# andrekuros/Multi-UAV-TA-gym-env

Hardware: AMD Instinct MI355X
Metric: env-steps/sec at N parallel envs, WPS_hard 16x32; 1/2/4/8 GPU (higher is better)
Workload: dtype f64

## Files before the change

include/muavta.h:

```cpp
#ifndef MUAVTA_H
#define MUAVTA_H

#include <stddef.h>
#include <stdint.h>

#ifdef __cplusplus
extern "C" {
#endif

#define MUAVTA_ABI_VERSION 1

enum { MUAVTA_R1 = 0, MUAVTA_R2 = 1, MUAVTA_E1 = 2, MUAVTA_F1 = 3, MUAVTA_F2 = 4, MUAVTA_T1 = 5, MUAVTA_T2 = 6 };
enum { MUAVTA_HOLD = 0, MUAVTA_REC = 1, MUAVTA_ATT = 2, MUAVTA_DEF = 3, MUAVTA_INT = 4, MUAVTA_DET = 5 };
enum { MUAVTA_EV_RESET_ALLOCATION = 0, MUAVTA_EV_NEW_THREAT = 1, MUAVTA_EV_AGENT_FAIL = 2,
       MUAVTA_EV_ESCORT_CREATED = 3, MUAVTA_EV_ESCORT_RETIRED = 4 };

enum {
  MUAVTA_OK = 0,
  MUAVTA_E_ARG = -1,
  MUAVTA_E_NO_DEVICE = -2,
  MUAVTA_E_HIP = -3,
  MUAVTA_E_CAPACITY = -4,
  MUAVTA_E_STATE = -5
};
// ... 194 lines not shown
  int32_t* n_stepped; uint8_t* park; double* reward_sum;
  int32_t max_steps, reserved;
} MuavtaRlRun;
int muavta_rl_run_device(MuavtaEnv* env, const MuavtaRlRun* run);
int muavta_step_run(MuavtaEnv* env, const int32_t* act_agent, const int32_t* act_index, int32_t gate, int32_t replan_interval, int32_t max_steps,
                    int32_t write_obs, int32_t* n_stepped, uint8_t* park, double* reward_sum);

int muavta_rollout(MuavtaEnv* env, const uint64_t* seeds, int32_t n_steps, int32_t replan_interval,
                   int32_t use_visibility, int32_t write_obs);

int muavta_set_lanes(MuavtaEnv* env, int32_t lanes);
int muavta_lanes(const MuavtaEnv* env, int32_t* mode, int32_t* allocated);
int muavta_rollout_metrics_back(MuavtaEnv* env, int32_t back, double* out);
int muavta_error_flags_back(MuavtaEnv* env, int32_t back, int32_t* flags );

int muavta_set_slot_cap(MuavtaEnv* env, int32_t cap);

int muavta_observe(MuavtaEnv* env, float* tasks, uint64_t* legal, uint8_t* pad, float* agents, float* flags);

int muavta_step_result(MuavtaEnv* env, double* reward, uint8_t* done);

int muavta_metrics(MuavtaEnv* env, double* out);

int muavta_get(MuavtaEnv* env, MuavtaField field, void* dst, size_t bytes);
int muavta_set(MuavtaEnv* env, MuavtaField field, const void* src, size_t bytes);

int muavta_get_state(MuavtaEnv* env, void* dst, size_t bytes);
int muavta_set_state(MuavtaEnv* env, const void* src, size_t bytes);

int muavta_lsap(int32_t device, const double* cost, int32_t n, int32_t nr, int32_t nc, int64_t* row, int64_t* col);
// ... 53 lines not shown
```

multi-uav-ta-gym-env_amd/batched.py:

```python
from __future__ import annotations

import ctypes as C
from typing import Optional, Sequence

import numpy as np

from . import native
from .native import MuavtaError
from .params import METRIC_KEYS, N_METRICS, N_SCALARS, MuavtaDims, MuavtaParams, params_from_config

F = {name: i for i, name in enumerate([
    "AGENT_POS", "AGENT_STATE", "AGENT_HEAD", "AGENT_QUEUE", "AGENT_NFT", "AGENT_NFP", "AGENT_CAPS", "AGENT_ATTACK_CAP",
    "AGENT_TYPE", "AGENT_NAME_IDX", "AGENT_DIST", "AGENT_MISC", "TASK_ID", "TASK_STATUS", "TASK_POS", "TASK_CUR",
    "TASK_ALLOC", "TASK_ORG_DONE", "TASK_META", "TASK_TIMES", "KNOWN", "THREAT_POS", "THREAT_META", "SCALARS",
    "OPEN_IDS", "EVENTS", "EVENT_LIST", "STAGED_ACTIONS", "ERROR", "RELEASE_LOG", "KNOWN_COUNT", "ESCORTS"])}


def _vp(a: Optional[np.ndarray]):
    return None if a is None else a.ctypes.data_as(C.c_void_p)


def _fp(a: np.ndarray):
    return C.c_void_p(a.ctypes.data)

# ... 589 lines not shown
        self._ck(self.L.muavta_metrics(self.h, _vp(m)))
        return m

    def set_slot_cap(self, cap: int = 0):
        self._ck(self.L.muavta_set_slot_cap(self.h, int(cap)))
        self.slot_cap = int(cap)

    def set_lanes(self, lanes: int = 0):
        self._ck(self.L.muavta_set_lanes(self.h, int(lanes)))

    def lanes(self):
        m, a = C.c_int32(), C.c_int32()
        self._ck(self.L.muavta_lanes(self.h, C.byref(m), C.byref(a)))
        return int(m.value), int(a.value)

    def error_flags(self, back: int = 0) -> np.ndarray:
        out = np.empty(self.n_envs, dtype=np.int32)
        self._ck(self.L.muavta_error_flags_back(self.h, int(back), _vp(out)))
        return out

    def rollout_metrics(self, back: int = 0) -> np.ndarray:
        m = np.empty((self.n_envs, N_METRICS), dtype=np.float64)
        if back:
            self._ck(self.L.muavta_rollout_metrics_back(self.h, int(back), _vp(m)))
            return m
        self._ck(self.L.muavta_rollout_metrics(self.h, _vp(m)))
        if self._esc_rows:
            for i, row in self._esc_rows.items():
                m[i] = row
        return m
# ... 129 lines not shown
```

multi-uav-ta-gym-env_amd/csrc/muavta_device.h:

```cpp
#pragma once
#include <hip/hip_runtime.h>
#include <cstddef>
#include <type_traits>

#include "muavta_state.h"

#define DEV __device__ __forceinline__
#define DEVN __device__ __noinline__

#ifndef MUAVTA_PACE_PRIO
#define MUAVTA_PACE_PRIO 4
#endif
#ifndef MUAVTA_PACE_HOLD
#define MUAVTA_PACE_HOLD 0
#endif
#ifndef MUAVTA_PACE_HOLD_WINDOW
#define MUAVTA_PACE_HOLD_WINDOW 48
#endif
#ifndef MUAVTA_PACE_HOLD_SLEEP
#define MUAVTA_PACE_HOLD_SLEEP 16
#endif
#ifndef MUAVTA_PACE_HOLD_POLLS
#define MUAVTA_PACE_HOLD_POLLS 256
#endif
// ... 94 lines not shown
  DEV unsigned long long* prof_lds() { return reinterpret_cast<unsigned long long*>(reinterpret_cast<unsigned char*>(&X) + sizeof(Scratch<TL>)); }
  DEV void prof_begin() { if (threadIdx.x < PROF_N) prof_lds()[threadIdx.x] = 0; if (threadIdx.x == 0) prof_lds()[PROF_N] = clock64(); lds_sync(); }
  DEV void prof_flush(int env) { lds_sync(); if (threadIdx.x < PROF_N && (g_prof_target < 0 || g_prof_target == env)) atomicAdd(&g_prof[threadIdx.x], prof_lds()[threadIdx.x]); }
#endif
  enum { A = TL::A, T = TL::T, H = TL::H, R = TL::R, E = TL::E, Q = TL::Q, KW = TL::KW };
  typedef EnvCold<TL> Cold;
  State& S;
  Cold& C;
  Scratch<TL>& X;
  double* rel_log = nullptr;
  const int32_t* more_agent = nullptr;
  const int32_t* more_index = nullptr;
  int more_cap = 0, more_pos = 0;
  int tnow;
  const DevParams& P;
  uint32_t* tape;
  int lane;
  const uint32_t* win_ptr;
  uint32_t win_len, win_stride;
  bool in_step = false;

  __device__ Sim(State& s, Cold& c, Scratch<TL>& x, const DevParams& p, uint32_t* t)
      : S(s), C(c), X(x), P(p), tape(t), lane(opaque_lane()), win_ptr(&s.rng_win[0][0]), win_len(8), win_stride(8), tnow(s.time_steps) {}
  static __device__ __forceinline__ int opaque_lane() {
    int l = threadIdx.x;
    asm volatile("" : "+v"(l));
    return l;
  }
  DEV void sync_clock() { tnow = S.time_steps; }
  DEV QueueSide<A, T, true>& qs() const {
    if constexpr (TL::SLIM) return static_cast<QueueSide<A, T, true>&>(C); else return static_cast<QueueSide<A, T, true>&>(S);
  }

  DEV void fail(int code) { if (S.error == 0) S.error = code; }
  enum { OBS_STATIC = 1 << 16 };
  DEV void obs_static_clear() { const int v = S.obs_rows; if (v > 0) S.obs_rows = v & (OBS_STATIC - 1); }
  DEV double speed_of(int t) const {
    return t == 0 ? P.speed[0] : t == 1 ? P.speed[1] : t == 2 ? P.speed[2] : t == 3 ? P.speed[3] : t == 4 ? P.speed[4]
         : t == 5 ? P.speed[5] : P.speed[6];
  }


#include "sim/rng.inc"
#include "sim/entities.inc"
#include "sim/reset.inc"
#include "sim/step.inc"
// ... 15 lines not shown
```

multi-uav-ta-gym-env_amd/csrc/muavta_kernels.hip:

```cpp
#include <hip/hip_runtime.h>
#include <dlfcn.h>
#include <rccl/rccl.h>

#include <cmath>
#include <cstdio>
#include <cstdlib>
#include <cstring>
#include <new>
#include <string>
#include <vector>

#include "muavta_device.h"

using namespace muavta;

namespace {

#define AS1 __attribute__((address_space(1)))
#define AS3 __attribute__((address_space(3)))
#define AS4 __attribute__((address_space(4)))
template <class T> __device__ __forceinline__ T* as_global(T* p) { return (T*)(AS1 T*)p; }

struct ObsPtrs {
  float* tasks;
// ... 14 lines not shown
  uint32_t* pace;
  PairPolicyDev pol;
};
enum { PACE_KEYS = 1 << 16 };
__device__ __forceinline__ const DevCtx& ctx_ref(const DevCtx* p) {
  const uint64_t b = (uint64_t)p;
  const uint32_t lo = __builtin_amdgcn_readfirstlane((uint32_t)b), hi = __builtin_amdgcn_readfirstlane((uint32_t)(b >> 32));
  return *(const DevCtx*)(const AS4 DevCtx*)(((uint64_t)hi << 32) | lo);
}
__device__ __forceinline__ ObsPtrs obs_ptrs(const DevCtx& c) {
  ObsPtrs o;
  o.tasks = as_global(c.O.tasks); o.legal = as_global(c.O.legal); o.pad = as_global(c.O.pad); o.agents = as_global(c.O.agents);
  o.flags = as_global(c.O.flags); o.reward = as_global(c.O.reward); o.done = as_global(c.O.done);
  return o;
}
template <class TL> __device__ __forceinline__ EnvState<TL>* blob_of(const DevCtx& c, int env) { return as_global(reinterpret_cast<EnvState<TL>*>(c.blobs)) + env; }
template <class TL> __device__ __forceinline__ EnvCold<TL>* cold_of(const DevCtx& c, int env) { return as_global(reinterpret_cast<EnvCold<TL>*>(c.cold)) + env; }
__device__ __forceinline__ uint32_t* tape_of(const DevCtx& c, int env) { return as_global(c.tapes) + (size_t)env * MUAVTA_RNG_STREAMS * MUAVTA_RNG_WORDS; }

template <class TL>
__device__ __forceinline__ void obs_for_env(Sim<TL>& sim, const DevParams& P, const ObsPtrs& O, int env, bool handle_buffer = true) {
  const size_t mt = (size_t)P.max_tasks, nA = (size_t)P.n_agents;
  sim.write_obs(O.tasks + (size_t)env * mt * 21, O.legal + (size_t)env * nA * ((mt + 63) >> 6), O.pad + (size_t)env * mt,
                O.agents + (size_t)env * nA * 9, O.flags + (size_t)env * 5, handle_buffer);
  if (threadIdx.x == 0) {
    O.reward[env] = sim.S.last_reward;
    O.done[env] = (uint8_t)((sim.S.terminated ? 1 : 0) | (sim.S.truncated ? 2 : 0));
  }
}

__device__ __forceinline__ void copy16(void* dst, const void* src, int bytes) {
// ... 16 lines not shown

#define smem muavta_smem
#ifdef MUAVTA_PROF
#define PROF_AT(sim, i) do { if (threadIdx.x == 0) { unsigned long long t_ = clock64(); (sim).prof_lds()[i] += t_ - (sim).prof_lds()[PROF_N]; (sim).prof_lds()[PROF_N] = t_; } } while (0)
#define PROF_EXTRA_LDS MUAVTA_PROF_LDS_BYTES
#else
#define PROF_AT(sim, i) do { } while (0)
#define PROF_EXTRA_LDS 0
#endif
#if MUAVTA_LDS_ZERO_REG
static __device__ __forceinline__ uint32_t lds_zero() { uint32_t z; asm volatile("v_mov_b32 %0, 0" : "=v"(z)); return z; }
#else
static __device__ __forceinline__ uint32_t lds_zero() { return 0u; }
#endif
#define KERNEL_LDS(TL) __shared__ __align__(16) unsigned char lds_own[Lds<TL>::bytes() + PROF_EXTRA_LDS]
static_assert(Lds<Tile16>::bytes() <= 10240, "Tile16 no longer fits 16 workgroups per CU");
static_assert(!MUAVTA_TILE24_SLIM || Lds<Tile24>::bytes() <= 10240, "Tile24 no longer fits 16 workgroups per CU");
static_assert(sizeof(EnvState<Tile16>) % 16 == 0 && sizeof(EnvState<Tile24>) % 16 == 0 && sizeof(EnvState<Tile64>) % 16 == 0, "blob copies move 16 B per lane");
static_assert(sizeof(EnvCold<Tile16>) % 16 == 0 && sizeof(EnvCold<Tile24>) % 16 == 0 && sizeof(EnvCold<Tile64>) % 16 == 0, "cold records are 16 B aligned");

#ifdef MUAVTA_MIN_WAVES
#define TILE_MIN_WAVES(TL) MUAVTA_MIN_WAVES
#else
#define TILE_MIN_WAVES(TL) TL::MIN_WAVES
#endif

struct GenrandTable {
  uint32_t v[624];
  constexpr GenrandTable() : v{} {
    uint32_t g = 19650218u;
    v[0] = g;
// ... 301 lines not shown
        if (G.R.reward_sum) as_global(G.R.reward_sum)[env] = rsum;
      }
      break;
    }
  }
  lds_sync();
  copy16(blob, L.S, sizeof(EnvState<TL>));
}

#ifndef MUAVTA_PHASE_ATTR
#define MUAVTA_PHASE_ATTR __forceinline__
#define MUAVTA_PHASE_INLINED 1
#else
#define MUAVTA_PHASE_INLINED 0
#endif
enum { PH_ALLOC = 1, PH_STEP = 2, PH_OBS = 4 };
template <class TL>
struct RecordPtrs {
  typename Sim<TL>::TokPtrs K;
  double* s_wps;
  ObsPtrs O;
  int n_envs;
};
struct RecBlob { uint32_t w[64]; };
__global__ void k_store_rec(RecBlob b, uint32_t* dst) { dst[threadIdx.x] = b.w[threadIdx.x]; }

template <class TL, bool REC, bool BL = false, bool PM = false>
__device__ MUAVTA_PHASE_ATTR void rollout_phase(const DevCtx* ctxp, unsigned char* lds_own, uint32_t lds_base, int env, int phases, int interval, int use_vis, int mode,
                                                const RecordPtrs<TL>& rec, int slot, int oslot) {
  const DevCtx& ctx = ctx_ref(ctxp);
#if MUAVTA_PHASE_INLINED
  Lds<TL> L(lds_own + lds_zero());
#else
  Lds<TL> L((unsigned char*)(AS3 unsigned char*)(uintptr_t)__builtin_amdgcn_readfirstlane(lds_base));
#endif
  Sim<TL> sim(*L.S, *cold_of<TL>(ctx, env), *L.X, ctx.P, tape_of(ctx, env));
  if (phases & PH_STEP) sim.step(true);
  if (phases & PH_OBS) {
    ObsPtrs O = obs_ptrs(ctx);
    int at = env;
    bool handle_buffer = true;
    if constexpr (REC) {
      if (oslot >= 0) {
        handle_buffer = false;
        O.tasks = as_global(rec.O.tasks); O.legal = as_global(rec.O.legal); O.pad = as_global(rec.O.pad); O.agents = as_global(rec.O.agents);
        O.flags = as_global(rec.O.flags); O.reward = as_global(rec.O.reward); O.done = as_global(rec.O.done);
        at = oslot * rec.n_envs + env;
      }
    }
    obs_for_env(sim, ctx.P, O, at, handle_buffer);
  }
// ... 3 lines not shown
                                       reinterpret_cast<unsigned char*>(L.S) + Lds<TL>::bytes() + PROF_EXTRA_LDS);
    else if constexpr (BL) sim.allocate_baseline(interval, use_vis, mode);
    else sim.allocate(interval, use_vis, mode);
    if (REC && rec.K.task_feats) {
      const typename Sim<TL>::TokPtrs K = global_tok_ptrs<TL>(rec.K);
      cold_sync();
      sim.tokens(K, slot * rec.n_envs + env);
      if (threadIdx.x == 0) as_global(rec.s_wps)[(size_t)slot * rec.n_envs + env] = sim.s_wps();
      lds_sync();
    }
  }
  PROF_AT(sim, 20);
}

template <class TL, bool REC, bool BL = false, bool PM = false>
__global__ __launch_bounds__(WG, PM ? (TILE_MIN_WAVES(TL) < 3 ? TILE_MIN_WAVES(TL) : 3) : TILE_MIN_WAVES(TL)) void k_rollout(const DevCtx* __restrict__ ctxp, const uint64_t* seeds, int n_steps, int interval, int use_vis,
                                                int mode, int write_obs, double* metrics, const uint32_t* seedbuf, const RecordPtrs<TL>* __restrict__ recp, int epoch, int env_base) {
  const DevCtx& ctx = ctx_ref(ctxp);
  const uint32_t rec_lo = __builtin_amdgcn_readfirstlane((uint32_t)(uint64_t)recp), rec_hi = __builtin_amdgcn_readfirstlane((uint32_t)((uint64_t)recp >> 32));
  const RecordPtrs<TL>& rec = *(const RecordPtrs<TL>*)(const AS4 RecordPtrs<TL>*)(((uint64_t)rec_hi << 32) | (uint64_t)rec_lo);
  const int env = env_base + blockIdx.x;
  __shared__ __align__(16) unsigned char lds_own[Lds<TL>::bytes() + PROF_EXTRA_LDS + (PM ? SCORED_EXTRA_LDS : 0)];
  Lds<TL> L(lds_own);
  EnvState<TL>* blob = blob_of<TL>(ctx, env);
  Sim<TL> sim(*L.S, *cold_of<TL>(ctx, env), *L.X, ctx.P, tape_of(ctx, env));
#ifndef MUAVTA_PACE_SCOPE
#if MUAVTA_PACE_HOLD
#define MUAVTA_PACE_SCOPE __HIP_MEMORY_SCOPE_AGENT
#else
#define MUAVTA_PACE_SCOPE __HIP_MEMORY_SCOPE_WORKGROUP
#endif
#endif
static_assert(MUAVTA_PACE_HOLD_POLLS > 0 && MUAVTA_PACE_HOLD_POLLS <= (1 << 16), "the hold loop of the pacing block must be poll-bounded");
#ifndef MUAVTA_PACE_EVERY
#define MUAVTA_PACE_EVERY 1
#endif
#if MUAVTA_PACE_PRIO
  constexpr bool PACED = TL::A <= 32 && !ABL(10);
  const uint32_t hw_id = __builtin_amdgcn_s_getreg(4 | (31 << 11)), xcc_id = __builtin_amdgcn_s_getreg(20 | (3 << 11));
  uint32_t* pace_row = as_global(ctx.pace) + ((((xcc_id & 15u) << 12) | ((hw_id >> 4) & 0xFFFu)) << 4);
// ... 24 lines not shown
          if (rec.K.task_feats) {
            const typename Sim<TL>::TokPtrs K = global_tok_ptrs<TL>(rec.K);
            const double fin = sim.s_wps();
            for (int sl = k - 1; sl < n_steps; sl++) {
              sim.tokens_pad(K, sl * rec.n_envs + env);
              if (threadIdx.x == 0) as_global(rec.s_wps)[(size_t)sl * rec.n_envs + env] = fin;
            }
          }
        }
        k = n_steps;
        continue;
      }
      ph = PH_STEP | (write_obs ? PH_OBS : 0) | (k < n_steps ? PH_ALLOC : 0);
    } else ph = (write_obs && !(REC && rec.O.tasks)) ? 0 : PH_OBS;
#if MUAVTA_PACE_PRIO
    uint32_t seen = 0;
    if (PACED && k >= 1 && k <= n_steps && (k & (MUAVTA_PACE_EVERY - 1)) == 0) {
      if (threadIdx.x == 0) __hip_atomic_store(pace_row + (hw_id & 15u), pace_tag | (uint32_t)k, __ATOMIC_RELAXED, MUAVTA_PACE_SCOPE);
      if (threadIdx.x < 16) seen = __hip_atomic_load(pace_row + threadIdx.x, __ATOMIC_RELAXED, MUAVTA_PACE_SCOPE);
    }
#endif
    if (ph) rollout_phase<TL, REC, BL, PM>(ctxp, lds_own, lds_base, env, ph, interval, use_vis, mode, rec, k < n_steps ? k : n_steps,
                                   (REC && rec.O.tasks && k >= 1 && k <= n_steps) ? k - 1 : -1);
#if MUAVTA_PACE_PRIO
    if (PACED && k >= 1 && k <= n_steps && (k & (MUAVTA_PACE_EVERY - 1)) == 0) {
      const bool behind_me = threadIdx.x < 16 && (seen >> 16) == (uint32_t)epoch && (seen & 0xFFFFu) < (uint32_t)k;
#if MUAVTA_PACE_PRIO == 4
      const int n_behind = __popcll(__ballot(behind_me));
      if (n_behind == 0) __builtin_amdgcn_s_setprio(3); else if (n_behind == 1) __builtin_amdgcn_s_setprio(2);
      else if (n_behind == 2) __builtin_amdgcn_s_setprio(1); else __builtin_amdgcn_s_setprio(0);
#else
      if (__ballot(behind_me) != 0ull) __builtin_amdgcn_s_setprio(0); else __builtin_amdgcn_s_setprio(MUAVTA_PACE_PRIO);
#endif
#if MUAVTA_PACE_HOLD
      for (int polls = 0; polls < MUAVTA_PACE_HOLD_POLLS; polls++) {
        const uint32_t st = seen & 0xFFFFu;
        const bool wait_for = threadIdx.x < 16 && (seen >> 16) == (uint32_t)epoch && st + MUAVTA_PACE_HOLD < (uint32_t)k &&
                              st + MUAVTA_PACE_HOLD_WINDOW >= (uint32_t)k;
        if (__ballot(wait_for) == 0ull) break;
        __builtin_amdgcn_s_sleep(MUAVTA_PACE_HOLD_SLEEP);
        if (threadIdx.x < 16) seen = __hip_atomic_load(pace_row + threadIdx.x, __ATOMIC_RELAXED, MUAVTA_PACE_SCOPE);
      }
#endif
    }
#endif
  }
#if MUAVTA_PACE_PRIO
  if (PACED && threadIdx.x == 0) __hip_atomic_store(pace_row + (hw_id & 15u), pace_tag | 0xFFFFu, __ATOMIC_RELAXED, MUAVTA_PACE_SCOPE);
  __builtin_amdgcn_s_setprio(0);
#endif
  if (REC && rec.K.task_feats) {
    if (threadIdx.x == 0) as_global(rec.s_wps)[(size_t)n_steps * rec.n_envs + env] = sim.s_wps();
  }
  sim.sync_clock();
  sim.metrics(as_global(metrics) + (size_t)env * MUAVTA_N_METRICS);
  lds_sync();
  copy16(blob, L.S, sizeof(EnvState<TL>));
#ifdef MUAVTA_PROF
  sim.prof_flush(env);
#endif
#ifdef MUAVTA_DIAG_TIMES
  if (threadIdx.x == 0 && env < 65536) {
    as_global(ctx.pace)[(1u << 19) + 65536 + env] = (uint32_t)__builtin_amdgcn_s_memrealtime();
    as_global(ctx.pace)[(1u << 19) + 131072 + env] = __builtin_amdgcn_s_getreg(4 | (31 << 11)) | (__builtin_amdgcn_s_getreg(20 | (3 << 11)) << 16);
  }
#endif
}

template <class TL>
__global__ __launch_bounds__(WG) void k_metrics(const DevCtx* __restrict__ ctxp, double* metrics) {
// ... 320 lines not shown
extern "C" int muavta_set_parts(MuavtaEnv* e, int32_t n_parts);
extern "C" int muavta_set_release_log(MuavtaEnv* e, int32_t enable);
extern "C" int muavta_create(const MuavtaParams* params, int32_t n_envs, int32_t device, MuavtaEnv** out);
extern "C" int muavta_destroy(MuavtaEnv* e);
extern "C" int muavta_set_slot_cap(MuavtaEnv* e, int32_t cap);
static int push_policy(MuavtaEnv* lane, const MuavtaEnv::HandleLevel& hl);

namespace {

template <class TL>
int launch_attr(MuavtaEnv* e) {
  size_t lds = Lds<TL>::bytes();
  e->lds_bytes = lds;
  if (lds > 48 * 1024) {
    const void* ks[] = {reinterpret_cast<const void*>(&k_reset<TL>), reinterpret_cast<const void*>(&k_step<TL>), reinterpret_cast<const void*>(&k_allocate<TL>),
                        reinterpret_cast<const void*>(&k_rollout<TL, false>), reinterpret_cast<const void*>(&k_rollout<TL, true>), reinterpret_cast<const void*>(&k_metrics<TL>), reinterpret_cast<const void*>(&k_observe<TL>),
                        reinterpret_cast<const void*>(&k_tokens<TL>), reinterpret_cast<const void*>(&k_call<TL>), reinterpret_cast<const void*>(&k_context<TL>),
                        reinterpret_cast<const void*>(&k_allocate<TL, true>), reinterpret_cast<const void*>(&k_rollout<TL, false, true>),
                        reinterpret_cast<const void*>(&k_pair_scores<TL>), reinterpret_cast<const void*>(&k_rollout<TL, false, false, true>)};
    for (const void* k : ks) HIPCHK(e, hipFuncSetAttribute(k, hipFuncAttributeMaxDynamicSharedMemorySize, (int)lds));
    HIPCHK(e, hipFuncSetAttribute(reinterpret_cast<const void*>(&k_allocate<TL, false, true>), hipFuncAttributeMaxDynamicSharedMemorySize, (int)lds + SCORED_EXTRA_LDS));
    HIPCHK(e, hipFuncSetAttribute(reinterpret_cast<const void*>(&k_allocate_scored<TL>), hipFuncAttributeMaxDynamicSharedMemorySize, (int)lds + SCORED_EXTRA_LDS));
  }
  return MUAVTA_OK;
}

#define DISPATCH(e, CALL)                    \
  switch ((e)->tile) {                       \
    case TK16: { typedef Tile16 TL; CALL; } break; \
    case TK24: { typedef Tile24 TL; CALL; } break; \
    default:   { typedef Tile64 TL; CALL; } break; \
// ... 870 lines not shown
    R.n_envs = e->n_envs;
    static_assert(sizeof(RecordPtrs<TL>) <= MuavtaEnv::REC_SLOT, "record-pointer slot too small");
    RecBlob blob;
    memset(&blob, 0, sizeof(blob));
    memcpy(&blob, &R, sizeof(R));
    hipLaunchKernelGGL(k_store_rec, dim3(1), dim3(64), 0, stream, blob, (uint32_t*)((char*)e->d_rec + MuavtaEnv::REC_SLOT));
    hipLaunchKernelGGL((k_rollout<TL, true>), dim3(n_launch), dim3(WG), extra_lds, stream, (const DevCtx*)e->d_ctx, ds,
                       n_steps, interval, use_vis, e->alloc_mode, write_obs, e->d_metrics, sb, (const RecordPtrs<TL>*)((char*)e->d_rec + MuavtaEnv::REC_SLOT), epoch, env_base);
  } else if (e->alloc_mode == MUAVTA_ALLOC_MLP_PAIR) {
    hipLaunchKernelGGL((k_rollout<TL, false, false, true>), dim3(n_launch), dim3(WG), extra_lds, stream, (const DevCtx*)e->d_ctx, ds,
                       n_steps, interval, use_vis, e->alloc_mode, write_obs, e->d_metrics, sb, (const RecordPtrs<TL>*)e->d_rec, epoch, env_base);
  } else if (e->alloc_mode >= MUAVTA_ALLOC_CAP_GREEDY) {
    hipLaunchKernelGGL((k_rollout<TL, false, true>), dim3(n_launch), dim3(WG), extra_lds, stream, (const DevCtx*)e->d_ctx, ds,
                       n_steps, interval, use_vis, e->alloc_mode, write_obs, e->d_metrics, sb, (const RecordPtrs<TL>*)e->d_rec, epoch, env_base);
  } else {
    hipLaunchKernelGGL((k_rollout<TL, false>), dim3(n_launch), dim3(WG), extra_lds, stream, (const DevCtx*)e->d_ctx, ds,
                       n_steps, interval, use_vis, e->alloc_mode, write_obs, e->d_metrics, sb, (const RecordPtrs<TL>*)e->d_rec, epoch, env_base);
  }
}
extern "C" {
static int rollout_impl(MuavtaEnv* e, const uint64_t* seeds, int32_t n_steps, int32_t interval, int32_t use_vis, int32_t write_obs, const MuavtaRecord* rec) {
  if (!e || n_steps < 0) return MUAVTA_E_ARG;
  if (!seeds && !e->did_reset) { e->err = "rollout without seeds before reset"; return MUAVTA_E_STATE; }
  DeviceScope scope_(e->device);
  if (seeds && e->hl.lanes_mode != 1) {
    bool want = e->hl.lanes_mode == 2;
    if (!want && e->n_rollouts) { want = hipEventQuery(e->ev1[(e->n_rollouts - 1) % MuavtaEnv::EV_RING]) == hipErrorNotReady; (void)hipGetLastError(); }
    if (want && ensure_twin(e) == MUAVTA_OK) flip_lanes(e);
  }
  MAIN_OP(e);
  const uint64_t* ds = nullptr;
  const uint32_t* sb = nullptr;
// ... 781 lines not shown
  if (lanes == 2) { int rc = ensure_twin(e); if (rc) { e->err = "muavta_set_lanes: the second lane could not be created: " + g_create_error; return rc; } }
  if (lanes == 1 && e->hl.twin) {
    muavta_destroy(e->hl.twin);
    e->hl.twin = nullptr;
  }
  e->hl.lanes_mode = lanes;
  return MUAVTA_OK;
}
int muavta_lanes(const MuavtaEnv* e, int32_t* mode, int32_t* allocated) {
  if (!e) return MUAVTA_E_ARG;
  if (mode) *mode = e->hl.lanes_mode;
  if (allocated) *allocated = e->hl.twin ? 2 : 1;
  return MUAVTA_OK;
}

int muavta_lsap(int32_t device, const double* cost, int32_t n, int32_t nr, int32_t nc, int64_t* row, int64_t* col) {
  return muavta_lsap_impl(device, cost, n, nr, nc, row, col, MUAVTA_LSAP_AUTO);
}
int muavta_lsap_impl(int32_t device, const double* cost, int32_t n, int32_t nr, int32_t nc, int64_t* row, int64_t* col, int32_t impl) {
  int ndev = 0;
  if (hipGetDeviceCount(&ndev) != hipSuccess || ndev < 1) { g_create_error = "muavta_lsap: no HIP device"; return MUAVTA_E_NO_DEVICE; }
  if (!cost || !row || !col || n < 1 || nr < 1 || nc < 1) { g_create_error = "muavta_lsap: bad arguments"; return MUAVTA_E_ARG; }
  int mn = nr < nc ? nr : nc, mx = nr < nc ? nc : nr;
  if (mn > Tile64::A || mx > Tile64::T) { g_create_error = "muavta_lsap: at most 64 x 128"; return MUAVTA_E_ARG; }
  for (size_t i = 0, m = (size_t)n * nr * nc; i < m; i++)
    if (std::isnan(cost[i]) || cost[i] == -INFINITY) { g_create_error = "muavta_lsap: matrix contains invalid numeric entries (NaN or -inf)"; return MUAVTA_E_ARG; }
  const bool fits_reg = mn <= TileLsapReg::A && mx <= TileLsapReg::T;
  if (impl < MUAVTA_LSAP_AUTO || impl > MUAVTA_LSAP_REGISTERS || (impl == MUAVTA_LSAP_REGISTERS && !fits_reg)) {
    g_create_error = "muavta_lsap_impl: unknown solver, or problem beyond 32 x 64 for the register solver"; return MUAVTA_E_ARG;
  }
// ... 112 lines not shown
```

multi-uav-ta-gym-env_amd/csrc/muavta_state.h:

```cpp
#pragma once
#include <stdint.h>

#include "../../include/muavta.h"


enum {
  MUAVTA_ERR_NONE = 0,
  MUAVTA_ERR_TASK_SLOTS = 1,
  MUAVTA_ERR_QUEUE = 2,
  MUAVTA_ERR_EVENTS = 3,
  MUAVTA_ERR_PENDING = 4,
  MUAVTA_ERR_POSITION = 5,
  MUAVTA_ERR_ESCORTS = 6,
  MUAVTA_ERR_LSAP = 7,
};

enum { TF_ESCORT = 1, TF_COUNTED = 2, TF_REACHED = 4, TF_ELIGIBLE = 8, TF_DEADLINE = 16,
       TF_KNOWN_ALL = 32  };

struct DevParams {
  int32_t n_agents, n_tasks , max_tasks , n_threats;
  int32_t n_agent_groups, agent_type[MUAVTA_MAX_GROUPS], agent_count[MUAVTA_MAX_GROUPS];
  int32_t n_task_groups, task_type[MUAVTA_MAX_GROUPS], task_count[MUAVTA_MAX_GROUPS];
  int32_t n_threat_groups, threat_type[MUAVTA_MAX_GROUPS], threat_count[MUAVTA_MAX_GROUPS];
// ... 3 lines not shown
      escort_required_agents , commit_horizon;
  uint32_t escort_mask;
  double speed[7];
  double threat_prob;
  double reward_norm_factor;
  double sense_sq_bound;
  double fail_rate, arrival_rate, dynamic_idle_penalty, sense_radius, miss_penalty, on_time_bonus,
      reassign_penalty, escort_radius, escort_requirement, escort_intercept_radius, mutual_support_radius;
  double rw[8];
  double escort_sq_bound;
  double inv_mts, inv_max_tasks;
  int32_t slot_cap;
  int32_t rw_plain;
};

template <int A_, int T_, int H_, int R_, int E_, int Q_, bool REGC_ = false, bool OTFC_ = false, bool SLIM_ = false>
struct Tile {
  static constexpr bool SLIM = SLIM_;
  static constexpr bool REGC = REGC_;
  static constexpr bool OTFC = OTFC_;
  static constexpr bool NO_COST_TILE = REGC_ || OTFC_;
  static constexpr int A = A_;
  static constexpr int T = T_;
  static constexpr int H = H_;
  static constexpr int R = R_;
  static constexpr int E = E_;
  static constexpr int Q = Q_;
  static constexpr int KW = (T_ + 31) / 32;
  static constexpr int MIN_WAVES = A_ > 32 ? 2 : 4;
  static_assert(A_ <= 64 && T_ <= 128 && H_ <= 64, "ids of agents / slots / threats are stored in int8");
};

// ... 4 lines not shown
template <> struct BucketMask<16> { typedef uint32_t type; };
template <> struct BucketMask<24> { typedef uint32_t type; };

typedef int8_t i8;
typedef int16_t i16;
typedef uint8_t u8;

template <int A, int T, bool HERE> struct QueueSide {
  double a_nfx[A], a_nfy[A], a_nft[A];
  double t_org[T], t_done[T];
  double area[3][3];
};
template <int A, int T> struct QueueSide<A, T, false> {};

template <class TL>
struct alignas(16) EnvCold : QueueSide<TL::A, TL::T, TL::SLIM> {
  enum { A = TL::A, T = TL::T, Q = TL::Q };
  double t_cur[6][T], t_alloc[6][T];
  double t_init[T], t_dtime[T];
  double a_qtime[A][Q];
  double obst[8][3];
};

template <class TL>
struct alignas(16) EnvState : QueueSide<TL::A, TL::T, !TL::SLIM> {
  enum { A = TL::A, T = TL::T, H = TL::H, R = TL::R, E = TL::E, Q = TL::Q, KW = TL::KW };
  double a_px[A], a_py[A];
  double a_dist[A];
  double a_caps[6][A];
  double t_px[T], t_py[T];
  double h_px[H], h_py[H];
// ... 42 lines not shown
      idle_reserve_steps, burst_region_toggle, escort_requests, escort_completed, escort_failed,
      escort_required_steps, escort_covered_steps, protection_breaches, threats_intercepted, recon_losses,
      escort_losses, mutual_support_engagements, protected_rec_completed;
  int32_t pending_reset, terminated, truncated, error, did_reset;
  int32_t last_plan_step, n_replans, n_calls;
  int32_t gate_step;
  uint32_t rng_idx[4];
  uint32_t rng_win[4][8];
  uint32_t rng_win_at[4];
  int32_t times_dirty;
  int32_t obs_rows;
  int32_t list_stale;
};

typedef Tile<16, 40, 16, 48, 40, 10, true> Tile16;
#ifndef MUAVTA_TILE24_SLIM
#define MUAVTA_TILE24_SLIM 1
#endif
typedef Tile<24, 48, 24, 88, 32, 12, true, false, MUAVTA_TILE24_SLIM != 0> Tile24;
typedef Tile<64, 128, 48, 128, 96, 12, true, true> Tile64;

#define MUAVTA_REL_ROW 29
#define MUAVTA_RNG_STREAMS 4
#define MUAVTA_RNG_WORDS 1248
```

multi-uav-ta-gym-env_amd/csrc/sim/entities.inc:

```
  DEV bool ref_valid(int id, int slot) const { return slot >= 0 && S.t_id[slot] == id; }
  DEV bool ref_retired(int id, int slot) const { return !ref_valid(id, slot) || S.t_status[slot] == 2; }
  DEV int head_id(int a) const { return S.a_qlen[a] > 0 ? S.a_qid[a][0] : 0; }
  DEV int queue_find(int a, int id) const {
    const int n = S.a_qlen[a];
    unsigned m = 0;
#pragma unroll
    for (int k = 0; k < Q; k++) m |= (unsigned)(S.a_qid[a][k] == id) << k;
    m &= (1u << n) - 1u;
    return m ? __ffs((int)m) - 1 : -1;
  }
  DEV void queue_erase(int a, int k) {
    const int n = S.a_qlen[a];
    for (int i = k; i + 1 < n; i++) {
      S.a_qid[a][i] = S.a_qid[a][i + 1];
      S.a_qslot[a][i] = S.a_qslot[a][i + 1];
    }
    for (int i = k; i + 1 < n; i += 4) {
      const int r = n - 1 - i;
      double t0 = 0, t1 = 0, t2 = 0, t3 = 0;
      if (r >= 1) t0 = C.a_qtime[a][i + 1];
      if (r >= 2) t1 = C.a_qtime[a][i + 2];
      if (r >= 3) t2 = C.a_qtime[a][i + 3];
      if (r >= 4) t3 = C.a_qtime[a][i + 4];
      if (r >= 1) C.a_qtime[a][i] = t0;
// ... 611 lines not shown
            }
          }
        }
      }
    }
    lds_sync();
    return __ballot(chg) != 0ull;
  }

  DEV void norm_vector(double& x, double& y) {
    double m = norm2(x, y);
    if (m == 0) { x = 0; y = 0; return; }
    const double r = frcp_nr(m);
    x = fdiv_r(x, m, r); y = fdiv_r(y, m, r);
  }
  DEV void avoid_obstacles(double px, double py, double mx, double my, double& ax, double& ay) {
    ax = 0.0; ay = 0.0;
    const double PI = 3.14159265358979323846;
    for (int o = 0; o < P.num_obstacles; o++) {
      double dx = C.obst[o][0] - px, dy = C.obst[o][1] - py;
      double d_zone = sqrt(dx * dx + dy * dy) - C.obst[o][2];
      if (d_zone < 40.0) {
        double nx = dx / d_zone, ny = dy / d_zone;
        double force = libm_log(fmax(1.05, d_zone));
        force = 0.5 / (1.0 - force);
        double ang = libm_atan2(my, mx) - libm_atan2(dy, dx);
        ang = fmod(ang + PI, 2.0 * PI) - PI;
        double rx, ry;
        if (ang > 0.0) { rx = ny; ry = -nx; } else { rx = -ny; ry = nx; }
        ax += rx * force;
        ay += ry * force;
      }
    }
  }
  DEV void random_position(int st, double min_distance, double own_range, bool contact_line, int area, bool check_obs,
                           double& ox, double& oy) {
    double limit_line = contact_line ? CONTACT_LINE : 0;
    for (int tries = 0; tries < 100; tries++) {
      double x, y;
      if (area >= 0) {
        double tlx = qs().area[area][0], tly = qs().area[area][1], w = qs().area[area][2];
// ... 57 lines not shown
```

multi-uav-ta-gym-env_amd/native.py:

```python
from __future__ import annotations

import ctypes as C
import os
import sys
import shutil
import subprocess

from .params import MuavtaDims, MuavtaParams

PKG_DIR = os.path.dirname(os.path.abspath(__file__))
CSRC = os.path.join(PKG_DIR, "csrc")
SO_PATH = os.environ.get("MUAVTA_SO") or os.path.join(PKG_DIR, "libmuavta.so")
HIPCC_FLAGS = ["--offload-arch=gfx950", "-O3", "-ldl", "-mllvm", "-disable-machine-licm",
                "-ffp-contract=off", "-std=c++17", "-fPIC", "-shared", "-Wno-unused-value", "-Wno-invalid-offsetof"]

EXPORTS = [
    "muavta_create", "muavta_destroy", "muavta_last_error", "muavta_dims", "muavta_reset", "muavta_step",
    "muavta_allocate", "muavta_step_staged", "muavta_rollout", "muavta_observe", "muavta_step_result",
    "muavta_metrics", "muavta_get", "muavta_set", "muavta_get_state", "muavta_set_state", "muavta_lsap",
    "muavta_avoid_obstacles", "muavta_device_ptrs", "muavta_last_kernel_ms", "muavta_sync",
    "muavta_rollout_metrics", "muavta_refresh_observation", "muavta_get_rng", "muavta_set_rng", "muavta_abi_sizes",
    "muavta_set_allocator", "muavta_tokens", "muavta_tokens_device", "muavta_set_release_log", "muavta_lsap_impl",
    "muavta_last_seed_ms", "muavta_call", "muavta_rollout_record", "muavta_comm_uid", "muavta_comm_init", "muavta_allreduce_metrics", "muavta_comm_destroy",
    "muavta_kernel_ms_history", "muavta_wait_stream", "muavta_set_parts", "muavta_part_range", "muavta_rollout_part", "muavta_allocate_part",
    "muavta_step_part", "muavta_observe_part", "muavta_wait_part", "muavta_domain_math", "muavta_domain_log", "muavta_domain_atan2", "muavta_step_lists",
    "muavta_allocate_scored", "muavta_allocate_scored_device", "muavta_rl_step_device", "muavta_launch_gaps_ms",
    "muavta_rl_run_device", "muavta_step_run", "muavta_set_lanes", "muavta_lanes", "muavta_rollout_metrics_back", "muavta_error_flags_back", "muavta_set_slot_cap", "muavta_context", "muavta_context_device",
    "muavta_set_pair_policy", "muavta_pair_scores", "muavta_pair_scores_device",
]


class MuavtaError(RuntimeError):
    pass


class MuavtaScored(C.Structure):
    _fields_ = [("kind", C.c_int32), ("max_tasks", C.c_int32), ("max_agents", C.c_int32), ("gate", C.c_int32), ("flags", C.c_int32),
                ("replan_interval", C.c_int32), ("use_visibility", C.c_int32), ("reserved0", C.c_int32),
                ("edge_scores", C.c_void_p), ("task_pri", C.c_void_p), ("reserved", C.c_void_p), ("selected", C.c_void_p),
                ("replanned", C.c_void_p)]


class MuavtaPairMlp(C.Structure):
# ... 116 lines not shown
    L.muavta_tokens.argtypes = [vp, i32, i32, i32] + [vp] * 10
    L.muavta_tokens_device.argtypes = [vp, i32, i32, i32] + [vp] * 10
    L.muavta_allocate_scored.argtypes = [vp, C.POINTER(MuavtaScored), vp, vp]
    L.muavta_allocate_scored_device.argtypes = [vp, C.POINTER(MuavtaScored)]
    L.muavta_rl_step_device.argtypes = [vp, C.POINTER(MuavtaRlStep)]
    L.muavta_rl_run_device.argtypes = [vp, C.POINTER(MuavtaRlRun)]
    L.muavta_step_run.argtypes = [vp, vp, vp, i32, i32, i32, i32, vp, vp, vp]
    L.muavta_set_lanes.argtypes = [vp, i32]
    L.muavta_set_slot_cap.argtypes = [vp, i32]
    L.muavta_context.argtypes = [vp, i32, i32, vp]
    L.muavta_context_device.argtypes = [vp, i32, i32, vp]
    L.muavta_set_pair_policy.argtypes = [vp, C.POINTER(MuavtaPairMlp)]
    L.muavta_pair_scores.argtypes = [vp, vp, vp]
    L.muavta_pair_scores_device.argtypes = [vp, vp, vp]
    L.muavta_lanes.argtypes = [vp, C.POINTER(i32), C.POINTER(i32)]
    L.muavta_rollout_metrics_back.argtypes = [vp, i32, vp]
    L.muavta_error_flags_back.argtypes = [vp, i32, vp]
    L.muavta_abi_sizes.argtypes = [C.POINTER(i32 * 3)]
    for name in EXPORTS:
        if name != "muavta_last_error":
            getattr(L, name).restype = C.c_int
    sizes = (i32 * 3)()
    L.muavta_abi_sizes(C.byref(sizes))
    if (sizes[0], sizes[1]) != (C.sizeof(MuavtaParams), C.sizeof(MuavtaDims)):
        raise MuavtaError(f"ABI layout mismatch: library {sizes[0]}/{sizes[1]} bytes vs binding "
                          f"{C.sizeof(MuavtaParams)}/{C.sizeof(MuavtaDims)} (MuavtaParams/MuavtaDims)")
    _LIB = L
    return L
```

Before: 236.6 million.

## Add lean Tile16 rollout with QueueSide in global memory for higher occupancy

Adds a Tile16Lean variant for the plain rollout kernel that keeps the QueueSide portion of env state in the global blob instead of LDS. This shrinks per-workgroup LDS so more workgroups fit per CU, and raises the launch-bounds minimum waves to 5. Queue accesses now go to global memory, which adds latency. It also computes the two atan2 calls in a nounroll loop to shrink code, moves the pace-row loads to after the phase, and adds an occupancy query API.

```diff
diff --git a/include/muavta.h b/include/muavta.h
--- a/include/muavta.h
+++ b/include/muavta.h
@@ -232,6 +232,8 @@
 int muavta_rollout_metrics_back(MuavtaEnv* env, int32_t back, double* out);
 int muavta_error_flags_back(MuavtaEnv* env, int32_t back, int32_t* flags );
 
+int muavta_rollout_occupancy(MuavtaEnv* env, int32_t* workgroups_per_cu);
+
 int muavta_set_slot_cap(MuavtaEnv* env, int32_t cap);
 
 int muavta_observe(MuavtaEnv* env, float* tasks, uint64_t* legal, uint8_t* pad, float* agents, float* flags);
diff --git a/multi-uav-ta-gym-env_amd/batched.py b/multi-uav-ta-gym-env_amd/batched.py
--- a/multi-uav-ta-gym-env_amd/batched.py
+++ b/multi-uav-ta-gym-env_amd/batched.py
@@ -627,6 +627,13 @@
         self._ck(self.L.muavta_lanes(self.h, C.byref(m), C.byref(a)))
         return int(m.value), int(a.value)
 
+    def rollout_occupancy(self) -> int:
+        if not hasattr(self.L, "muavta_rollout_occupancy"):
+            raise MuavtaError("this build of libmuavta.so has no muavta_rollout_occupancy")
+        n = C.c_int32()
+        self._ck(self.L.muavta_rollout_occupancy(self.h, C.byref(n)))
+        return int(n.value)
+
     def error_flags(self, back: int = 0) -> np.ndarray:
         out = np.empty(self.n_envs, dtype=np.int32)
         self._ck(self.L.muavta_error_flags_back(self.h, int(back), _vp(out)))
diff --git a/multi-uav-ta-gym-env_amd/csrc/muavta_device.h b/multi-uav-ta-gym-env_amd/csrc/muavta_device.h
--- a/multi-uav-ta-gym-env_amd/csrc/muavta_device.h
+++ b/multi-uav-ta-gym-env_amd/csrc/muavta_device.h
@@ -132,6 +132,7 @@
   int more_cap = 0, more_pos = 0;
   int tnow;
   const DevParams& P;
+  QueueSide<A, T, true>* QB = nullptr;
   uint32_t* tape;
   int lane;
   const uint32_t* win_ptr;
@@ -140,14 +141,22 @@
 
   __device__ Sim(State& s, Cold& c, Scratch<TL>& x, const DevParams& p, uint32_t* t)
       : S(s), C(c), X(x), P(p), tape(t), lane(opaque_lane()), win_ptr(&s.rng_win[0][0]), win_len(8), win_stride(8), tnow(s.time_steps) {}
+  __device__ Sim(State& s, Cold& c, Scratch<TL>& x, const DevParams& p, uint32_t* t, int lane_)
+      : S(s), C(c), X(x), P(p), tape(t), lane(lane_), win_ptr(&s.rng_win[0][0]), win_len(8), win_stride(8), tnow(s.time_steps) {}
   static __device__ __forceinline__ int opaque_lane() {
     int l = threadIdx.x;
     asm volatile("" : "+v"(l));
     return l;
   }
+  static __device__ __forceinline__ uint32_t wave_lane() {
+    uint32_t l = __builtin_amdgcn_mbcnt_hi(~0u, __builtin_amdgcn_mbcnt_lo(~0u, 0u));
+    asm volatile("" : "+v"(l));
+    return l;
+  }
   DEV void sync_clock() { tnow = S.time_steps; }
   DEV QueueSide<A, T, true>& qs() const {
-    if constexpr (TL::SLIM) return static_cast<QueueSide<A, T, true>&>(C); else return static_cast<QueueSide<A, T, true>&>(S);
+    if constexpr (TL::LEAN) return *(QueueSide<A, T, true>*)(__attribute__((address_space(1))) QueueSide<A, T, true>*)QB;
+    else if constexpr (TL::SLIM) return static_cast<QueueSide<A, T, true>&>(C); else return static_cast<QueueSide<A, T, true>&>(S);
   }
 
   DEV void fail(int code) { if (S.error == 0) S.error = code; }
diff --git a/multi-uav-ta-gym-env_amd/csrc/muavta_kernels.hip b/multi-uav-ta-gym-env_amd/csrc/muavta_kernels.hip
--- a/multi-uav-ta-gym-env_amd/csrc/muavta_kernels.hip
+++ b/multi-uav-ta-gym-env_amd/csrc/muavta_kernels.hip
@@ -52,7 +52,15 @@
   o.flags = as_global(c.O.flags); o.reward = as_global(c.O.reward); o.done = as_global(c.O.done);
   return o;
 }
-template <class TL> __device__ __forceinline__ EnvState<TL>* blob_of(const DevCtx& c, int env) { return as_global(reinterpret_cast<EnvState<TL>*>(c.blobs)) + env; }
+template <class TL> __device__ __forceinline__ EnvState<TL>* blob_of(const DevCtx& c, int env) {
+  if constexpr (TL::LEAN) {
+    typedef EnvState<typename TL::Full> FS;
+    return reinterpret_cast<EnvState<TL>*>(reinterpret_cast<unsigned char*>(as_global(reinterpret_cast<FS*>(c.blobs)) + env) + offsetof(FS, a_px));
+  } else return as_global(reinterpret_cast<EnvState<TL>*>(c.blobs)) + env;
+}
+template <class TL> __device__ __forceinline__ QueueSide<TL::A, TL::T, true>* qs_of(const DevCtx& c, int env) {
+  return reinterpret_cast<QueueSide<TL::A, TL::T, true>*>(as_global(reinterpret_cast<EnvState<typename TL::Full>*>(c.blobs)) + env);
+}
 template <class TL> __device__ __forceinline__ EnvCold<TL>* cold_of(const DevCtx& c, int env) { return as_global(reinterpret_cast<EnvCold<TL>*>(c.cold)) + env; }
 __device__ __forceinline__ uint32_t* tape_of(const DevCtx& c, int env) { return as_global(c.tapes) + (size_t)env * MUAVTA_RNG_STREAMS * MUAVTA_RNG_WORDS; }
 
@@ -99,7 +107,22 @@
 static __device__ __forceinline__ uint32_t lds_zero() { return 0u; }
 #endif
 #define KERNEL_LDS(TL) __shared__ __align__(16) unsigned char lds_own[Lds<TL>::bytes() + PROF_EXTRA_LDS]
+static_assert(Lds<Tile16Lean>::bytes() <= 8192, "the plain rollout of Tile16 no longer fits 20 workgroups per CU");
 static_assert(Lds<Tile16>::bytes() <= 10240, "Tile16 no longer fits 16 workgroups per CU");
+template <class TL> struct LeanImage {
+  typedef typename TL::Full FT;
+  static constexpr size_t offset() { return offsetof(EnvState<FT>, a_px); }
+  static constexpr bool ok() {
+    return offsetof(EnvState<TL>, a_px) == 0 && offset() % 8 == 0 && offset() + sizeof(EnvState<TL>) <= sizeof(EnvState<FT>) &&
+           offsetof(EnvState<FT>, list_stale) - offset() == offsetof(EnvState<TL>, list_stale) &&
+           offsetof(EnvState<FT>, esc_mask) - offset() == offsetof(EnvState<TL>, esc_mask) &&
+           offsetof(EnvState<FT>, a_qslot) - offset() == offsetof(EnvState<TL>, a_qslot) &&
+           offsetof(EnvState<FT>, t_bucket) - offset() == offsetof(EnvState<TL>, t_bucket) &&
+           sizeof(EnvCold<TL>) == sizeof(EnvCold<FT>) && offsetof(EnvCold<TL>, obst) == offsetof(EnvCold<FT>, obst) &&
+           sizeof(QueueSide<TL::A, TL::T, true>) <= offset();
+  }
+};
+static_assert(LeanImage<Tile16Lean>::ok(), "Tile16Lean is not the image of Tile16 behind QueueSide");
 static_assert(!MUAVTA_TILE24_SLIM || Lds<Tile24>::bytes() <= 10240, "Tile24 no longer fits 16 workgroups per CU");
 static_assert(sizeof(EnvState<Tile16>) % 16 == 0 && sizeof(EnvState<Tile24>) % 16 == 0 && sizeof(EnvState<Tile64>) % 16 == 0, "blob copies move 16 B per lane");
 static_assert(sizeof(EnvCold<Tile16>) % 16 == 0 && sizeof(EnvCold<Tile24>) % 16 == 0 && sizeof(EnvCold<Tile64>) % 16 == 0, "cold records are 16 B aligned");
@@ -431,6 +454,13 @@
 #else
 #define MUAVTA_PHASE_INLINED 0
 #endif
+template <class TL> struct RolloutTile { typedef TL type; };
+template <> struct RolloutTile<Tile16> { typedef Tile16Lean type; };
+#ifdef MUAVTA_MIN_WAVES
+#define ROLLOUT_MIN_WAVES(TL, REC, BL, PM) ((PM) && MUAVTA_MIN_WAVES > 3 ? 3 : MUAVTA_MIN_WAVES)
+#else
+#define ROLLOUT_MIN_WAVES(TL, REC, BL, PM) ((PM) ? (TL::MIN_WAVES < 3 ? TL::MIN_WAVES : 3) : TL::LEAN ? 5 : TL::MIN_WAVES)
+#endif
 enum { PH_ALLOC = 1, PH_STEP = 2, PH_OBS = 4 };
 template <class TL>
 struct RecordPtrs {
@@ -451,7 +481,9 @@
 #else
   Lds<TL> L((unsigned char*)(AS3 unsigned char*)(uintptr_t)__builtin_amdgcn_readfirstlane(lds_base));
 #endif
-  Sim<TL> sim(*L.S, *cold_of<TL>(ctx, env), *L.X, ctx.P, tape_of(ctx, env));
+  constexpr bool FIVE = ROLLOUT_MIN_WAVES(TL, REC, BL, PM) > TL::MIN_WAVES;
+  Sim<TL> sim(*L.S, *cold_of<TL>(ctx, env), *L.X, ctx.P, tape_of(ctx, env), FIVE ? (int)Sim<TL>::wave_lane() : Sim<TL>::opaque_lane());
+  if constexpr (TL::LEAN) sim.QB = qs_of<TL>(ctx, env);
   if (phases & PH_STEP) sim.step(true);
   if (phases & PH_OBS) {
     ObsPtrs O = obs_ptrs(ctx);
@@ -485,7 +517,7 @@
 }
 
 template <class TL, bool REC, bool BL = false, bool PM = false>
-__global__ __launch_bounds__(WG, PM ? (TILE_MIN_WAVES(TL) < 3 ? TILE_MIN_WAVES(TL) : 3) : TILE_MIN_WAVES(TL)) void k_rollout(const DevCtx* __restrict__ ctxp, const uint64_t* seeds, int n_steps, int interval, int use_vis,
+__global__ __launch_bounds__(WG, ROLLOUT_MIN_WAVES(TL, REC, BL, PM)) void k_rollout(const DevCtx* __restrict__ ctxp, const uint64_t* seeds, int n_steps, int interval, int use_vis,
                                                 int mode, int write_obs, double* metrics, const uint32_t* seedbuf, const RecordPtrs<TL>* __restrict__ recp, int epoch, int env_base) {
   const DevCtx& ctx = ctx_ref(ctxp);
   const uint32_t rec_lo = __builtin_amdgcn_readfirstlane((uint32_t)(uint64_t)recp), rec_hi = __builtin_amdgcn_readfirstlane((uint32_t)((uint64_t)recp >> 32));
@@ -495,6 +527,7 @@
   Lds<TL> L(lds_own);
   EnvState<TL>* blob = blob_of<TL>(ctx, env);
   Sim<TL> sim(*L.S, *cold_of<TL>(ctx, env), *L.X, ctx.P, tape_of(ctx, env));
+  if constexpr (TL::LEAN) sim.QB = qs_of<TL>(ctx, env);
 #ifndef MUAVTA_PACE_SCOPE
 #if MUAVTA_PACE_HOLD
 #define MUAVTA_PACE_SCOPE __HIP_MEMORY_SCOPE_AGENT
@@ -549,17 +582,18 @@
       ph = PH_STEP | (write_obs ? PH_OBS : 0) | (k < n_steps ? PH_ALLOC : 0);
     } else ph = (write_obs && !(REC && rec.O.tasks)) ? 0 : PH_OBS;
 #if MUAVTA_PACE_PRIO
-    uint32_t seen = 0;
     if (PACED && k >= 1 && k <= n_steps && (k & (MUAVTA_PACE_EVERY - 1)) == 0) {
-      if (threadIdx.x == 0) __hip_atomic_store(pace_row + (hw_id & 15u), pace_tag | (uint32_t)k, __ATOMIC_RELAXED, MUAVTA_PACE_SCOPE);
-      if (threadIdx.x < 16) seen = __hip_atomic_load(pace_row + threadIdx.x, __ATOMIC_RELAXED, MUAVTA_PACE_SCOPE);
+      if (Sim<TL>::wave_lane() == 0) __hip_atomic_store(pace_row + (hw_id & 15u), pace_tag | (uint32_t)k, __ATOMIC_RELAXED, MUAVTA_PACE_SCOPE);
     }
 #endif
     if (ph) rollout_phase<TL, REC, BL, PM>(ctxp, lds_own, lds_base, env, ph, interval, use_vis, mode, rec, k < n_steps ? k : n_steps,
                                    (REC && rec.O.tasks && k >= 1 && k <= n_steps) ? k - 1 : -1);
 #if MUAVTA_PACE_PRIO
     if (PACED && k >= 1 && k <= n_steps && (k & (MUAVTA_PACE_EVERY - 1)) == 0) {
-      const bool behind_me = threadIdx.x < 16 && (seen >> 16) == (uint32_t)epoch && (seen & 0xFFFFu) < (uint32_t)k;
+      const uint32_t pl = Sim<TL>::wave_lane();
+      uint32_t seen = 0;
+      if (pl < 16) seen = __hip_atomic_load(pace_row + pl, __ATOMIC_RELAXED, MUAVTA_PACE_SCOPE);
+      const bool behind_me = pl < 16 && (seen >> 16) == (uint32_t)epoch && (seen & 0xFFFFu) < (uint32_t)k;
 #if MUAVTA_PACE_PRIO == 4
       const int n_behind = __popcll(__ballot(behind_me));
       if (n_behind == 0) __builtin_amdgcn_s_setprio(3); else if (n_behind == 1) __builtin_amdgcn_s_setprio(2);
@@ -574,21 +608,24 @@
                               st + MUAVTA_PACE_HOLD_WINDOW >= (uint32_t)k;
         if (__ballot(wait_for) == 0ull) break;
         __builtin_amdgcn_s_sleep(MUAVTA_PACE_HOLD_SLEEP);
-        if (threadIdx.x < 16) seen = __hip_atomic_load(pace_row + threadIdx.x, __ATOMIC_RELAXED, MUAVTA_PACE_SCOPE);
+        if (pl < 16) seen = __hip_atomic_load(pace_row + pl, __ATOMIC_RELAXED, MUAVTA_PACE_SCOPE);
       }
 #endif
     }
 #endif
   }
 #if MUAVTA_PACE_PRIO
-  if (PACED && threadIdx.x == 0) __hip_atomic_store(pace_row + (hw_id & 15u), pace_tag | 0xFFFFu, __ATOMIC_RELAXED, MUAVTA_PACE_SCOPE);
+  if (PACED && Sim<TL>::wave_lane() == 0) __hip_atomic_store(pace_row + (hw_id & 15u), pace_tag | 0xFFFFu, __ATOMIC_RELAXED, MUAVTA_PACE_SCOPE);
   __builtin_amdgcn_s_setprio(0);
 #endif
   if (REC && rec.K.task_feats) {
     if (threadIdx.x == 0) as_global(rec.s_wps)[(size_t)n_steps * rec.n_envs + env] = sim.s_wps();
   }
-  sim.sync_clock();
-  sim.metrics(as_global(metrics) + (size_t)env * MUAVTA_N_METRICS);
+  {
+    Sim<TL> fin(*L.S, *cold_of<TL>(ctx, env), *L.X, ctx.P, tape_of(ctx, env));
+    if constexpr (TL::LEAN) fin.QB = qs_of<TL>(ctx, env);
+    fin.metrics(as_global(metrics) + (size_t)env * MUAVTA_N_METRICS);
+  }
   lds_sync();
   copy16(blob, L.S, sizeof(EnvState<TL>));
 #ifdef MUAVTA_PROF
@@ -939,7 +976,7 @@
   e->lds_bytes = lds;
   if (lds > 48 * 1024) {
     const void* ks[] = {reinterpret_cast<const void*>(&k_reset<TL>), reinterpret_cast<const void*>(&k_step<TL>), reinterpret_cast<const void*>(&k_allocate<TL>),
-                        reinterpret_cast<const void*>(&k_rollout<TL, false>), reinterpret_cast<const void*>(&k_rollout<TL, true>), reinterpret_cast<const void*>(&k_metrics<TL>), reinterpret_cast<const void*>(&k_observe<TL>),
+                        reinterpret_cast<const void*>(&k_rollout<typename RolloutTile<TL>::type, false>), reinterpret_cast<const void*>(&k_rollout<TL, true>), reinterpret_cast<const void*>(&k_metrics<TL>), reinterpret_cast<const void*>(&k_observe<TL>),
                         reinterpret_cast<const void*>(&k_tokens<TL>), reinterpret_cast<const void*>(&k_call<TL>), reinterpret_cast<const void*>(&k_context<TL>),
                         reinterpret_cast<const void*>(&k_allocate<TL, true>), reinterpret_cast<const void*>(&k_rollout<TL, false, true>),
                         reinterpret_cast<const void*>(&k_pair_scores<TL>), reinterpret_cast<const void*>(&k_rollout<TL, false, false, true>)};
@@ -1840,8 +1877,9 @@
     hipLaunchKernelGGL((k_rollout<TL, false, true>), dim3(n_launch), dim3(WG), extra_lds, stream, (const DevCtx*)e->d_ctx, ds,
                        n_steps, interval, use_vis, e->alloc_mode, write_obs, e->d_metrics, sb, (const RecordPtrs<TL>*)e->d_rec, epoch, env_base);
   } else {
-    hipLaunchKernelGGL((k_rollout<TL, false>), dim3(n_launch), dim3(WG), extra_lds, stream, (const DevCtx*)e->d_ctx, ds,
-                       n_steps, interval, use_vis, e->alloc_mode, write_obs, e->d_metrics, sb, (const RecordPtrs<TL>*)e->d_rec, epoch, env_base);
+    typedef typename RolloutTile<TL>::type RT;
+    hipLaunchKernelGGL((k_rollout<RT, false>), dim3(n_launch), dim3(WG), extra_lds, stream, (const DevCtx*)e->d_ctx, ds,
+                       n_steps, interval, use_vis, e->alloc_mode, write_obs, e->d_metrics, sb, (const RecordPtrs<RT>*)e->d_rec, epoch, env_base);
   }
 }
 extern "C" {
@@ -2653,6 +2691,23 @@
   return MUAVTA_OK;
 }
 
+}
+template <class TL>
+static hipError_t rollout_occupancy(const MuavtaEnv* e, int* n) {
+  if (e->alloc_mode == MUAVTA_ALLOC_MLP_PAIR) return hipOccupancyMaxActiveBlocksPerMultiprocessor(n, k_rollout<TL, false, false, true>, WG, 0);
+  if (e->alloc_mode >= MUAVTA_ALLOC_CAP_GREEDY) return hipOccupancyMaxActiveBlocksPerMultiprocessor(n, k_rollout<TL, false, true>, WG, 0);
+  return hipOccupancyMaxActiveBlocksPerMultiprocessor(n, k_rollout<typename RolloutTile<TL>::type, false>, WG, 0);
+}
+extern "C" {
+int muavta_rollout_occupancy(MuavtaEnv* e, int32_t* workgroups_per_cu) {
+  if (!e || !workgroups_per_cu) return MUAVTA_E_ARG;
+  DeviceScope scope_(e->device);
+  int n = 0;
+  DISPATCH(e, HIPCHK(e, rollout_occupancy<TL>(e, &n)));
+  *workgroups_per_cu = n;
+  return MUAVTA_OK;
+}
+
 int muavta_lsap(int32_t device, const double* cost, int32_t n, int32_t nr, int32_t nc, int64_t* row, int64_t* col) {
   return muavta_lsap_impl(device, cost, n, nr, nc, row, col, MUAVTA_LSAP_AUTO);
 }
diff --git a/multi-uav-ta-gym-env_amd/csrc/muavta_state.h b/multi-uav-ta-gym-env_amd/csrc/muavta_state.h
--- a/multi-uav-ta-gym-env_amd/csrc/muavta_state.h
+++ b/multi-uav-ta-gym-env_amd/csrc/muavta_state.h
@@ -41,8 +41,11 @@
   int32_t rw_plain;
 };
 
-template <int A_, int T_, int H_, int R_, int E_, int Q_, bool REGC_ = false, bool OTFC_ = false, bool SLIM_ = false>
+template <int A_, int T_, int H_, int R_, int E_, int Q_, bool REGC_ = false, bool OTFC_ = false, bool SLIM_ = false, bool LEAN_ = false>
 struct Tile {
+  static constexpr bool LEAN = LEAN_;
+  typedef Tile<A_, T_, H_, R_, E_, Q_, REGC_, OTFC_, LEAN_ ? false : SLIM_, false> Full;
+  static_assert(!LEAN_ || SLIM_, "a lean view keeps QueueSide out of LDS");
   static constexpr bool SLIM = SLIM_;
   static constexpr bool REGC = REGC_;
   static constexpr bool OTFC = OTFC_;
@@ -77,7 +80,7 @@
 template <int A, int T> struct QueueSide<A, T, false> {};
 
 template <class TL>
-struct alignas(16) EnvCold : QueueSide<TL::A, TL::T, TL::SLIM> {
+struct alignas(16) EnvCold : QueueSide<TL::A, TL::T, TL::SLIM && !TL::LEAN> {
   enum { A = TL::A, T = TL::T, Q = TL::Q };
   double t_cur[6][T], t_alloc[6][T];
   double t_init[T], t_dtime[T];
@@ -150,6 +153,7 @@
 };
 
 typedef Tile<16, 40, 16, 48, 40, 10, true> Tile16;
+typedef Tile<16, 40, 16, 48, 40, 10, true, false, true, true> Tile16Lean;
 #ifndef MUAVTA_TILE24_SLIM
 #define MUAVTA_TILE24_SLIM 1
 #endif
diff --git a/multi-uav-ta-gym-env_amd/csrc/sim/entities.inc b/multi-uav-ta-gym-env_amd/csrc/sim/entities.inc
--- a/multi-uav-ta-gym-env_amd/csrc/sim/entities.inc
+++ b/multi-uav-ta-gym-env_amd/csrc/sim/entities.inc
@@ -649,6 +649,9 @@
     const double r = frcp_nr(m);
     x = fdiv_r(x, m, r); y = fdiv_r(y, m, r);
   }
+#ifndef MUAVTA_ATAN2_ONE_COPY
+#define MUAVTA_ATAN2_ONE_COPY 1
+#endif
   DEV void avoid_obstacles(double px, double py, double mx, double my, double& ax, double& ay) {
     ax = 0.0; ay = 0.0;
     const double PI = 3.14159265358979323846;
@@ -659,7 +662,17 @@
         double nx = dx / d_zone, ny = dy / d_zone;
         double force = libm_log(fmax(1.05, d_zone));
         force = 0.5 / (1.0 - force);
+#if MUAVTA_ATAN2_ONE_COPY
+        double a_mov = 0.0, a_obs = 0.0;
+#pragma nounroll
+        for (int k = 0; k < 2; k++) {
+          const double a = libm_atan2(k ? dy : my, k ? dx : mx);
+          if (k) a_obs = a; else a_mov = a;
+        }
+        double ang = a_mov - a_obs;
+#else
         double ang = libm_atan2(my, mx) - libm_atan2(dy, dx);
+#endif
         ang = fmod(ang + PI, 2.0 * PI) - PI;
         double rx, ry;
         if (ang > 0.0) { rx = ny; ry = -nx; } else { rx = -ny; ry = nx; }
diff --git a/multi-uav-ta-gym-env_amd/native.py b/multi-uav-ta-gym-env_amd/native.py
--- a/multi-uav-ta-gym-env_amd/native.py
+++ b/multi-uav-ta-gym-env_amd/native.py
@@ -26,7 +26,7 @@
     "muavta_step_part", "muavta_observe_part", "muavta_wait_part", "muavta_domain_math", "muavta_domain_log", "muavta_domain_atan2", "muavta_step_lists",
     "muavta_allocate_scored", "muavta_allocate_scored_device", "muavta_rl_step_device", "muavta_launch_gaps_ms",
     "muavta_rl_run_device", "muavta_step_run", "muavta_set_lanes", "muavta_lanes", "muavta_rollout_metrics_back", "muavta_error_flags_back", "muavta_set_slot_cap", "muavta_context", "muavta_context_device",
-    "muavta_set_pair_policy", "muavta_pair_scores", "muavta_pair_scores_device",
+    "muavta_set_pair_policy", "muavta_pair_scores", "muavta_pair_scores_device", "muavta_rollout_occupancy",
 ]
 
 
@@ -173,11 +173,13 @@
     L.muavta_pair_scores.argtypes = [vp, vp, vp]
     L.muavta_pair_scores_device.argtypes = [vp, vp, vp]
     L.muavta_lanes.argtypes = [vp, C.POINTER(i32), C.POINTER(i32)]
+    if hasattr(L, "muavta_rollout_occupancy"):
+        L.muavta_rollout_occupancy.argtypes = [vp, C.POINTER(i32)]
     L.muavta_rollout_metrics_back.argtypes = [vp, i32, vp]
     L.muavta_error_flags_back.argtypes = [vp, i32, vp]
     L.muavta_abi_sizes.argtypes = [C.POINTER(i32 * 3)]
     for name in EXPORTS:
-        if name != "muavta_last_error":
+        if name != "muavta_last_error" and (name != "muavta_rollout_occupancy" or hasattr(L, name)):
             getattr(L, name).restype = C.c_int
     sizes = (i32 * 3)()
     L.muavta_abi_sizes(C.byref(sizes))
```

After: 235.6 million. About the same (-0.4%).
